# mborhi/CoMA-UNet

Hardware: AMD Instinct MI355X
Metric: volumes/sec (train fwd+bwd) at 128^3 bf16 (higher is better)
Workload: dtype bf16; 1 GPU; CoMA-UNet train step (fwd + RoiMSE/RnC loss + bwd + all-reduce + AdamW), 128^3 volumes, batch 2/GPU, 6-dim covariates (BASELINE configs[3]); global_batch=2, parallelism=dp1, launch=hipGraph replay of the whole step

## Files before the change

coma_unet_amd/csrc/conv_mfma.hip:

```cpp
#include "conv_mfma.h"
#include <type_traits>

template <typename T> struct elem;
template <> struct elem<bf16_t> { static constexpr int EPB = 8; };
template <> struct elem<float> { static constexpr int EPB = 4; };

__device__ __forceinline__ f32x16_t mma_piece(const uint4& a, const uint4& b, f32x16_t acc, bf16_t) {
  return __builtin_amdgcn_mfma_f32_32x32x16_bf16(*reinterpret_cast<const bf16x8_t*>(&a), *reinterpret_cast<const bf16x8_t*>(&b), acc, 0, 0, 0);
}
__device__ __forceinline__ f32x16_t mma_piece(const uint4& a, const uint4& b, f32x16_t acc, float) {
  acc = __builtin_amdgcn_mfma_f32_32x32x2f32(__uint_as_float(a.x), __uint_as_float(b.x), acc, 0, 0, 0);
  acc = __builtin_amdgcn_mfma_f32_32x32x2f32(__uint_as_float(a.y), __uint_as_float(b.y), acc, 0, 0, 0);
  acc = __builtin_amdgcn_mfma_f32_32x32x2f32(__uint_as_float(a.z), __uint_as_float(b.z), acc, 0, 0, 0);
  acc = __builtin_amdgcn_mfma_f32_32x32x2f32(__uint_as_float(a.w), __uint_as_float(b.w), acc, 0, 0, 0);
  return acc;
}

struct GatherP {
  const void* x; int ldx; long sbx; int Di, Hi, Wi, C;
  void* y; int ldy; long sby; int Do, Ho, Wo, N;
  const void* w; long wsb;
  const float* bias; int bsb;
  int k, stride, flip;
  int Mz, My, Mx;
  int ksplit;
  float* part; long part_sb;
  int accum;
  double2* stats; int stats_inst;
};

__device__ __forceinline__ int swz(int row, int chunk) { return (row << 2) | (chunk ^ ((row >> 2) & 3)); }

template <int BN, int MODE, typename T = bf16_t>
__global__ __launch_bounds__(256, 2) void conv_mfma_gather_k(GatherP p) {
  constexpr int EPB = elem<T>::EPB, CKL = 4 * EPB, LCK = EPB == 8 ? 5 : 4;
  constexpr int BM = (BN == 128) ? 128 : 256;
  constexpr int WAVES_N = (BN == 128) ? 2 : 1;
  constexpr int NT = BN / 32 / WAVES_N;
  constexpr int MT = 2;
  constexpr int A_PIECES = BM * 4 / 256;
  constexpr int B_PIECES = (BN * 4 + 255) / 256;
  extern __shared__ __attribute__((aligned(16))) char smem[];
  uint4* ldsA = reinterpret_cast<uint4*>(smem);
  uint4* ldsB = ldsA + 2 * BM * 4;
  int* rowoff = reinterpret_cast<int*>(ldsB + 2 * BN * 4);

  const int tid = threadIdx.x, lane = tid & 63, wid = tid >> 6;
  const int wm = wid / WAVES_N, wn = wid % WAVES_N;
  const int b = blockIdx.z;
  int nblk, cls = 0, ysl = blockIdx.y, ksi = 0;
  if (p.ksplit > 1) { ksi = ysl % p.ksplit; ysl /= p.ksplit; }
  if (MODE == 1) { cls = ysl & 7; nblk = ysl >> 3; } else { nblk = ysl; }
  const int n0 = nblk * BN;
  const int pz = (cls >> 2) & 1, py = (cls >> 1) & 1, px = cls & 1;
  const long Mtot = (long)p.Mz * p.My * p.Mx;
  const long m0 = (long)blockIdx.x * BM;
  const T* xb = static_cast<const T*>(p.x) + (long)b * p.sbx;
  const T* wb = static_cast<const T*>(p.w) + (long)b * p.wsb;
  const int pad = (p.k - 1) >> 1;

  const int chunk = tid & 3;
  int rz[A_PIECES], ry[A_PIECES], rx[A_PIECES];
#pragma unroll
  for (int i = 0; i < A_PIECES; ++i) {
    const int row = (tid >> 2) + 64 * i;
    const long m = m0 + row;
    if (m < Mtot) {
      const int mx = (int)(m % p.Mx), my = (int)((m / p.Mx) % p.My), mz = (int)(m / ((long)p.Mx * p.My));
      if (MODE == 0) { rz[i] = mz * p.stride - pad; ry[i] = my * p.stride - pad; rx[i] = mx * p.stride - pad; }
      else { rz[i] = mz; ry[i] = my; rx[i] = mx; }
      if (chunk == 0) {
        int off;
        if (MODE == 0) off = (int)(m * p.ldy);
        else {
          const int oz = 2 * mz + pz, oy = 2 * my + py, ox = 2 * mx + px;
          off = (oz < p.Do && oy < p.Ho && ox < p.Wo) ? (((oz * p.Ho + oy) * p.Wo + ox) * p.ldy) : -1;
        }
        rowoff[row] = off;
      }
    } else {
      rz[i] = ry[i] = rx[i] = -(1 << 20);
      if (chunk == 0) rowoff[row] = -1;
    }
  }

  const int cchunks = p.C >> LCK;
  int ntaps;
  if (MODE == 0) ntaps = p.k * p.k * p.k; else ntaps = (1 + pz) * (1 + py) * (1 + px);
  const int nsteps_all = ntaps * cchunks;
  const int s_begin = p.ksplit > 1 ? (int)((long)nsteps_all * ksi / p.ksplit) : 0;
  const int s_end = p.ksplit > 1 ? (int)((long)nsteps_all * (ksi + 1) / p.ksplit) : nsteps_all;
  const int nsteps = s_end - s_begin;
  if (nsteps <= 0) return;

  uint4 ra[A_PIECES], rb[B_PIECES];
  const int l_nx = MODE == 0 ? p.k : 1 + px, l_ny = MODE == 0 ? p.k : 1 + py;
  int l_t = s_begin / cchunks, l_cc = s_begin % cchunks;
  int l_jx = l_t % l_nx, l_jy = (l_t / l_nx) % l_ny, l_jz = l_t / (l_nx * l_ny);
  auto load_step = [&](int) {
    const int t = l_t, cc = l_cc;
    int dz, dy, dx, wtap;
    if (MODE == 0) {
      dz = l_jz; dy = l_jy; dx = l_jx;
      wtap = p.flip ? (ntaps - 1 - t) : t;
    } else {
      const int jx = l_jx, jy = l_jy, jz = l_jz;
      const int tx = px ? (jx ? 2 : 0) : 1, ty = py ? (jy ? 2 : 0) : 1, tz = pz ? (jz ? 2 : 0) : 1;
      dx = px ? (jx ? 0 : 1) : 0; dy = py ? (jy ? 0 : 1) : 0; dz = pz ? (jz ? 0 : 1) : 0;
      wtap = (tz * 3 + ty) * 3 + tx;
    }
    const int c0 = cc * CKL + chunk * EPB;
#pragma unroll
    for (int i = 0; i < A_PIECES; ++i) {
      const int iz = rz[i] + dz, iy = ry[i] + dy, ix = rx[i] + dx;
      const bool ok = (unsigned)iz < (unsigned)p.Di && (unsigned)iy < (unsigned)p.Hi && (unsigned)ix < (unsigned)p.Wi;
      ra[i] = make_uint4(0, 0, 0, 0);
      if (ok) ra[i] = *reinterpret_cast<const uint4*>(xb + (long)((iz * p.Hi + iy) * p.Wi + ix) * p.ldx + c0);
    }
#pragma unroll
    for (int i = 0; i < B_PIECES; ++i) {
      const int piece = tid + 256 * i;
      const int n = piece >> 2;
      rb[i] = make_uint4(0, 0, 0, 0);
      if (n < BN) rb[i] = *reinterpret_cast<const uint4*>(wb + ((long)wtap * p.N + n0 + n) * p.C + c0);
    }
    if (++l_cc == cchunks) {
      l_cc = 0; ++l_t;
      if (++l_jx == l_nx) { l_jx = 0; if (++l_jy == l_ny) { l_jy = 0; ++l_jz; } }
    }
  };
  auto store_step = [&](int buf) {
#pragma unroll
    for (int i = 0; i < A_PIECES; ++i) ldsA[buf * BM * 4 + swz((tid >> 2) + 64 * i, chunk)] = ra[i];
#pragma unroll
    for (int i = 0; i < B_PIECES; ++i) {
      const int piece = tid + 256 * i;
      const int n = piece >> 2;
      if (n < BN) ldsB[buf * BN * 4 + swz(n, chunk)] = rb[i];
    }
  };

  f32x16_t acc[MT][NT];
#pragma unroll
  for (int i = 0; i < MT; ++i)
#pragma unroll
    for (int j = 0; j < NT; ++j)
#pragma unroll
      for (int e = 0; e < 16; ++e) acc[i][j][e] = 0.f;

  load_step(0);
  store_step(0);
  __syncthreads();
  const int fr = lane & 31, fh = lane >> 5;
  int cur = 0;
  for (int step = 0; step < nsteps; ++step) {
    if (step + 1 < nsteps) load_step(step + 1);
    const uint4* A = ldsA + cur * BM * 4;
    const uint4* B = ldsB + cur * BN * 4;
#pragma unroll
    for (int ks = 0; ks < 2; ++ks) {
      uint4 af[MT], bfr[NT];
#pragma unroll
      for (int i = 0; i < MT; ++i) af[i] = A[swz(wm * 64 + i * 32 + fr, ks * 2 + fh)];
#pragma unroll
      for (int j = 0; j < NT; ++j) bfr[j] = B[swz(wn * (NT * 32) + j * 32 + fr, ks * 2 + fh)];
#pragma unroll
      for (int i = 0; i < MT; ++i)
#pragma unroll
        for (int j = 0; j < NT; ++j) acc[i][j] = mma_piece(af[i], bfr[j], acc[i][j], T());
    }
    if (step + 1 < nsteps) store_step(cur ^ 1);
    __syncthreads();
    cur ^= 1;
  }

  T* yb = static_cast<T*>(p.y) + (long)b * p.sby;
  const bool do_stats = p.stats != nullptr;
  float st_s[NT], st_q[NT];
#pragma unroll
  for (int j = 0; j < NT; ++j) {
    const int n = n0 + wn * (NT * 32) + j * 32 + fr;
    const float bv = p.bias ? p.bias[b * p.bsb + n] : 0.f;
    st_s[j] = 0.f; st_q[j] = 0.f;
#pragma unroll
    for (int i = 0; i < MT; ++i) {
#pragma unroll
      for (int e = 0; e < 16; ++e) {
        const int row = wm * 64 + i * 32 + (e & 3) + 8 * (e >> 2) + 4 * fh;
        const int off = rowoff[row];
        if (off >= 0) {
          if (p.ksplit > 1) atomicAdd(p.part + (long)b * p.part_sb + (long)(off / p.ldy) * p.N + n, acc[i][j][e]);
          else {
            const T o = static_cast<T>(acc[i][j][e] + bv + (p.accum ? static_cast<float>(yb[off + n]) : 0.f));
            yb[off + n] = o;
            if (do_stats) { const float r = static_cast<float>(o); st_s[j] += r; st_q[j] = fmaf(r, r, st_q[j]); }
          }
        }
      }
    }
  }
  if (do_stats) {
    __syncthreads();
    float* red = reinterpret_cast<float*>(smem);
#pragma unroll
    for (int j = 0; j < NT; ++j) {
      float a = st_s[j], c = st_q[j];
      a += __shfl_xor(a, 32, 64); c += __shfl_xor(c, 32, 64);
      if (fh == 0) { red[((wid * NT + j) * 32 + fr) * 2] = a; red[((wid * NT + j) * 32 + fr) * 2 + 1] = c; }
    }
    __syncthreads();
    for (int t = tid; t < BN; t += 256) {
      const int twn = t / (NT * 32), tj = (t / 32) % NT, tfr = t & 31;
      double a = 0.0, c = 0.0;
      for (int w = 0; w < 4 / WAVES_N; ++w) {
        const int wv_ = w * WAVES_N + twn;
        a += (double)red[((wv_ * NT + tj) * 32 + tfr) * 2]; c += (double)red[((wv_ * NT + tj) * 32 + tfr) * 2 + 1];
      }
      stat_add(p.stats, p.stats_inst ? p.stats_inst : 1, p.N, p.stats_inst ? b : 0, n0 + t, a, c);
    }
  }
}

template <typename T>
__global__ __launch_bounds__(256) void gather_finalize_k(const float* __restrict__ part, long part_sb, T* __restrict__ y, int ldy,
                                                         long sby, int N, long V, const float* __restrict__ bias, int bsb, int accum) {
  const int b = blockIdx.y;
  const long total = V * N;
  for (long e = (long)blockIdx.x * 256 + threadIdx.x; e < total; e += (long)gridDim.x * 256) {
    const long v = e / N; const int n = (int)(e - v * N);
    T* dst = y + (long)b * sby + v * ldy + n;
    *dst = static_cast<T>(part[(long)b * part_sb + e] + (bias ? bias[b * bsb + n] : 0.f) + (accum ? static_cast<float>(*dst) : 0.f));
  }
}

struct HaloP {
  const void* x; int ldx; long sbx; int D, H, W, C;
  void* y; int ldy; long sby; int N;
  const void* w; long wsb;
  const float* bias; int bsb;
  int flip, vecx, vecw;
  int ntx, nty, ntz;
};

template <int CPR> __device__ __forceinline__ int hswz(int row, int chunk) {
  if (CPR == 4) return (row << 2) | (chunk ^ ((row >> 2) & 3));
  return (row << 1) | (chunk ^ ((row >> 3) & 1));
}

template <int CK, int LX, int VEC, typename T = bf16_t>
__global__ __launch_bounds__(256, 2) void conv_mfma_halo_k(HaloP p) {
  constexpr int EPB = elem<T>::EPB;
  static_assert(EPB == 8 || VEC == 1, "fp32 staging is vector-only");
  constexpr int TX = 1 << LX, RY = 32 / TX;
  constexpr int TY = 4 * RY, TZ = 2;
  constexpr int HX = TX + 2, HY = TY + 2, HZ = TZ + 2, HV = HX * HY * HZ;
  constexpr int CPR = CK / EPB;
  constexpr int KS = CPR / 2;
  extern __shared__ __attribute__((aligned(16))) char smem[];
  uint4* Hl = reinterpret_cast<uint4*>(smem);
  uint4* Wl = Hl + HV * CPR;
  const int tid = threadIdx.x, lane = tid & 63, wid = tid >> 6;
  const int b = blockIdx.z, n0 = blockIdx.y * 32;
  int tix, tiy, tiz;
  if (!tile_coords(xcd_remap(blockIdx.x, gridDim.x), p.ntx, p.nty, p.ntz, tix, tiy, tiz)) return;
  const int x0 = tix * TX, y0 = tiy * TY, z0 = tiz * TZ;
  const T* xb = static_cast<const T*>(p.x) + (long)b * p.sbx;
  const T* wb = static_cast<const T*>(p.w) + (long)b * p.wsb;
  const int fr = lane & 31, fh = lane >> 5;

  f32x16_t acc[2];
#pragma unroll
  for (int i = 0; i < 2; ++i)
#pragma unroll
    for (int e = 0; e < 16; ++e) acc[i][e] = 0.f;
// ... 1888 lines not shown
  TconvP q;
  q.x = x->data; q.ldx = (int)x->ld; q.sbx = x->sb; q.D = x->D; q.H = x->H; q.W = x->W; q.C = x->C;
  q.y = y->data; q.ldy = (int)y->ld; q.sby = y->sb; q.Do = y->D; q.Ho = y->H; q.Wo = y->W; q.N = y->C;
  q.w = wk; q.wsb = d->per_sample_w ? 27L * y->C * x->C : 0;
  q.bias = bias; q.bsb = d->per_sample_w ? y->C : 0;
  q.xbytes = (unsigned)((unsigned long long)t_vox(x) * x->ld * sizeof(T));
  q.wbytes = (unsigned)(27ull * y->C * x->C * sizeof(T));
  q.accum = accum;
  const int nblk_n = y->C / 32;
  const TileRun r = tile_run(q.D, q.H, q.W, 32, 4, 2, 512, nblk_n * x->B);
  q.ntx = r.ntx; q.nty = r.nty; q.ntz = r.ntz; q.ids_total = r.ids_total; q.ids_per_block = r.ids_per_block;
  q.stats = nullptr; q.stats_inst = stats_inst;
  static const bool fuse_stats = getenv("COMA_TCONV_NO_STATS") == nullptr;
  if (stats && !accum && fuse_stats) { q.stats = stats; *stats_chunks = 1; }
  const size_t lds = (size_t)(33 * 5 * 3 + 14 * 32) * 80;
  coma_set_kernel_tag("conv_mfma_tconv_k<%s, %d>", sizeof(T) == 2 ? "__bf16" : "float", q.stats ? 1 : 0);
  const dim3 grid((unsigned)r.gx, (unsigned)nblk_n, (unsigned)x->B);
  if (q.stats) { set_max_lds<conv_mfma_tconv_k<T, true>>(); hipLaunchKernelGGL((conv_mfma_tconv_k<T, true>), grid, dim3(256), lds, s, q); }
  else { set_max_lds<conv_mfma_tconv_k<T, false>>(); hipLaunchKernelGGL((conv_mfma_tconv_k<T, false>), grid, dim3(256), lds, s, q); }
  COMA_LAUNCH_CHECK();
  return 0;
}

bool conv_mfma_supported(const coma_conv_desc* d, const coma_tensor* x, const coma_tensor* y) {
  if (x->dtype != COMA_BF16 || y->dtype != COMA_BF16) return false;
  if ((long)t_vox(x) * x->ld >= (1L << 31) || (long)t_vox(y) * y->ld >= (1L << 31)) return false;
  if (halo_ok(d, x, y)) return true;
  if (pw_ok(d, x, y)) return true;
  if (x->C % 32 || y->C % 32) return false;
  if (x->ld % 8 || y->ld % 8 || x->sb % 8 || y->sb % 8) return false;
  if (x->data && !aligned16(x->data)) return false;
  if ((long)t_vox(x) * x->ld >= (1L << 31) || (long)t_vox(y) * y->ld >= (1L << 31)) return false;
  if (d->form == 1 && d->stride == 2 && d->ksize != 3) return false;
  return true;
}

static bool f32_halo_ok(const coma_conv_desc* d, const coma_tensor* x, const coma_tensor* y) {
  if (x->W < 16 && x->C % 32 == 0 && y->C % 32 == 0) return false;
  return d->ksize == 3 && d->stride == 1 && x->W >= 8 && (long)x->H * x->W >= 32 && x->C % 16 == 0 && y->C >= 16 &&
         x->ld % 4 == 0 && x->sb % 4 == 0 && (!x->data || aligned16(x->data)) && (unsigned long long)t_vox(x) * x->ld * 4 < 0x7fff0000ull;
}
bool conv_f32mfma_supported(const coma_conv_desc* d, const coma_tensor* x, const coma_tensor* y) {
  if (x->dtype != COMA_F32 || y->dtype != COMA_F32) return false;
  if ((long)t_vox(x) * x->ld >= (1L << 31) || (long)t_vox(y) * y->ld >= (1L << 31)) return false;
  if (thin16f_ok(d, x, y)) return true;
  if (f32_halo_ok(d, x, y)) return true;
  if (x->C % 16 || y->C % 32) return false;
  if (x->ld % 4 || y->ld % 4 || x->sb % 4 || y->sb % 4) return false;
  if (x->data && !aligned16(x->data)) return false;
  if (d->form == 1 && d->stride == 2 && d->ksize != 3) return false;
  return true;
}

static int gather_ksplit(long blocks, int nsteps, bool f32) {
  if (f32) {
    if (blocks >= 192 || nsteps < 8) return 1;
    long ks = 256 / blocks;
    if (ks > 8) ks = 8;
    if (ks > nsteps / 4) ks = nsteps / 4;
    return ks < 2 ? 1 : (int)ks;
  }
  if (blocks >= 384 || nsteps < 16) return 1;
  long ks = 512 / blocks;
  if (ks > 8) ks = 8;
  if (ks > nsteps / 4) ks = nsteps / 4;
  return ks < 2 ? 1 : (int)ks;
}

struct GatherGrid { long gx, gy; int ksplit; };
static GatherGrid gather_grid(int BN, int mode, long Mtot, int N, int B, int taps, int C, bool f32) {
  const int BM = BN == 128 ? 128 : 256, LCK = f32 ? 4 : 5;
  GatherGrid g;
  g.gx = (Mtot + BM - 1) / BM; g.gy = (long)(N / BN) * (mode == 1 ? 8 : 1);
  g.ksplit = gather_ksplit(g.gx * g.gy * B, (mode == 1 ? 1 : taps) * (C >> LCK), f32);
  return g;
}

template <int BN, typename T>
static int launch_gather(const GatherP& p0, int mode, int B, hipStream_t s, void* ws, size_t ws_bytes, int ws_zeroed,
                         double2* stats, int stats_inst, int* stats_chunks) {
  GatherP p = p0;
  constexpr int BM = (BN == 128) ? 128 : 256;
  constexpr int LCK = elem<T>::EPB == 8 ? 5 : 4;
  const size_t lds = (size_t)2 * (BM + BN) * 64 + BM * 4;
  const GatherGrid g = gather_grid(BN, mode, (long)p.Mz * p.My * p.Mx, p.N, B, p.k * p.k * p.k, p.C, LCK == 4);
  const unsigned gx = (unsigned)g.gx, gy = (unsigned)g.gy;
  const long Vout = (long)p.Do * p.Ho * p.Wo;
  p.ksplit = g.ksplit;
  p.part = nullptr; p.part_sb = 0;
  if (p.ksplit > 1 && ws && ws_bytes >= sizeof(float) * (size_t)B * Vout * p.N) {
    p.part = (float*)ws; p.part_sb = Vout * p.N;
    if (!ws_zeroed && hipMemsetAsync(ws, 0, sizeof(float) * (size_t)B * Vout * p.N, s) != hipSuccess) { coma_set_error("conv split-K memset failed"); return 2; }
  } else p.ksplit = 1;
  p.stats = nullptr; p.stats_inst = stats_inst;
  if (stats && p.ksplit == 1 && !p.accum) { p.stats = stats; *stats_chunks = 1; }
  dim3 grid(gx, gy * p.ksplit, (unsigned)B);
  coma_set_kernel_tag("conv_mfma_gather_k<%d, %d, %s>", BN, mode, LCK == 4 ? "float" : "__bf16");
  if (mode == 0) hipLaunchKernelGGL((conv_mfma_gather_k<BN, 0, T>), grid, dim3(256), lds, s, p);
  else hipLaunchKernelGGL((conv_mfma_gather_k<BN, 1, T>), grid, dim3(256), lds, s, p);
  COMA_LAUNCH_CHECK();
  if (p.ksplit > 1) {
    long nb = (Vout * p.N + 255) / 256;
    if (nb > 1024) nb = 1024;
    hipLaunchKernelGGL(gather_finalize_k<T>, dim3((unsigned)nb, (unsigned)B), dim3(256), 0, s, (const float*)p.part, p.part_sb, (T*)p.y, p.ldy,
                       p.sby, p.N, Vout, p.bias, p.bsb, p.accum);
    COMA_LAUNCH_CHECK();
  }
  return 0;
}

template <int CK, int LX, int VEC, typename T>
static int launch_halo(const HaloP& p0, int B, hipStream_t s) {
  HaloP p = p0;
  constexpr int TX = 1 << LX, RY = 32 / TX, TY = 4 * RY, TZ = 2;
  constexpr int HV = (TX + 2) * (TY + 2) * (TZ + 2);
  p.ntx = (p.W + TX - 1) / TX; p.nty = (p.H + TY - 1) / TY; p.ntz = (p.D + TZ - 1) / TZ;
  const size_t lds = (size_t)(HV + 9 * 32) * CK * sizeof(T);
  set_max_lds<conv_mfma_halo_k<CK, LX, VEC, T>, 96>();
  dim3 grid((unsigned)(p.ntx * p.nty * ((p.ntz + 7) / 8) * 8), (unsigned)((p.N + 31) / 32), (unsigned)B);
  coma_set_kernel_tag("conv_mfma_halo_k<%d, %d, %d, %s>", CK, LX, VEC, sizeof(T) == 4 ? "float" : "__bf16");
  hipLaunchKernelGGL((conv_mfma_halo_k<CK, LX, VEC, T>), grid, dim3(256), lds, s, p);
  COMA_LAUNCH_CHECK();
  return 0;
}

static int duo_mode() {
  static const int mode = getenv("COMA_NO_DUO") != nullptr ? 0 : getenv("COMA_DUO_C32_ONLY") != nullptr ? 1 : 2;
  return mode;
}
static size_t duo_frag_bytes(const coma_conv_desc* d, const coma_tensor* x, const coma_tensor* y) {
  if (duo_mode() < 2 || x->dtype != COMA_BF16 || d->ksize != 3 || d->stride != 1 || x->W < 16) return 0;
  if (x->C < 64 || x->C % 16 || y->C % 32) return 0;
  return (size_t)(d->per_sample_w ? x->B : 1) * 27 * y->C * x->C * 2;
}

static bool duo_wide_ok(const coma_conv_desc* d, const coma_tensor* x, const coma_tensor* y) {
  if (duo_frag_bytes(d, x, y) == 0 || x->C <= 32 || x->C % 32) return false;
  const bool vecx = x->ld % 8 == 0 && x->sb % 8 == 0 && aligned16(x->data);
  const bool st16 = y->ld % 8 == 0 && y->sb % 8 == 0 && aligned16(y->data);
  return vecx && st16 && (unsigned long long)t_vox(x) * x->ld * sizeof(bf16_t) < 0x7fff0000ull &&
         x->D <= 510 && x->H <= 510 && x->W <= 510;
}

template <typename T>
static int conv_mfma_halo(const coma_conv_desc* d, const coma_tensor* x, const void* wk, const float* bias,
                          const coma_tensor* y, hipStream_t s, double2* stats = nullptr, int stats_inst = 0,
                          int* stats_chunks = nullptr, void* ws = nullptr, size_t ws_bytes = 0, bool wk_frag = false) {
  constexpr int EPB = elem<T>::EPB;
  constexpr bool F32 = EPB == 4;
  HaloP p;
  p.x = x->data; p.ldx = (int)x->ld; p.sbx = x->sb; p.D = x->D; p.H = x->H; p.W = x->W; p.C = x->C;
  p.y = y->data; p.ldy = (int)y->ld; p.sby = y->sb; p.N = y->C;
  p.w = wk; p.wsb = d->per_sample_w ? 27L * y->C * x->C : 0;
  p.bias = bias; p.bsb = d->per_sample_w ? y->C : 0;
  p.flip = d->form == 1;
  p.vecx = x->ld % EPB == 0 && x->sb % EPB == 0 && aligned16(x->data);
  p.vecw = x->C % EPB == 0 && aligned16(wk);
  const bool thin = !F32 && x->C <= 16;
  const int lx = x->W >= 32 ? 5 : (x->W >= 16 ? 4 : 3);
  const bool vec = p.vecx && p.vecw && x->C % (4 * EPB) == 0 && (unsigned long long)t_vox(x) * x->ld * sizeof(T) < 0x7fff0000ull;
  if (F32) COMA_CHECK(vec, "conv_mfma(fp32): operands must allow 16-byte channel pieces (C %% 16 == 0, aligned)");
  if constexpr (!F32) {
    static const bool thin16_on = []{ const char* e = getenv("COMA_THIN16"); return !(e && e[0] == '0'); }();
    const unsigned long long xb_ = (unsigned long long)t_vox(x) * x->ld * sizeof(T);
    if (thin16_on && thin && lx == 5 && y->C <= (x->C > 8 ? 16 : 32) && p.vecx && xb_ < 0x7fff0000ull) {
      Thin16P q;
      q.x = (const bf16_t*)p.x; q.ldx = p.ldx; q.sbx = p.sbx; q.D = p.D; q.H = p.H; q.W = p.W; q.C = p.C;
      q.y = (bf16_t*)p.y; q.ldy = p.ldy; q.sby = p.sby; q.N = p.N; q.w = (const bf16_t*)p.w; q.wsb = p.wsb; q.bias = p.bias; q.bsb = p.bsb;
      q.flip = p.flip; q.xbytes = (unsigned)xb_;
      q.st8 = y->ld % 4 == 0 && y->sb % 4 == 0 && (((uintptr_t)y->data) & 7) == 0;
      const TileRun r = tile_run(q.D, q.H, q.W, 32, 4, 2, 1024, x->B);
      q.ntx = r.ntx; q.nty = r.nty; q.ntz = r.ntz; q.ids_total = r.ids_total; q.ids_per_block = r.ids_per_block;
      q.stats = nullptr; q.stats_inst = stats_inst;
      if (stats) { q.stats = stats; *stats_chunks = 1; }
      dim3 grid((unsigned)r.gx, 1, (unsigned)x->B);
      const bool c16 = q.C > 8, n32 = q.N > 16;
      size_t lds = (size_t)34 * 6 * 4 * (c16 ? 32 : 16);
      if (lds < (size_t)27 * q.N * q.C * 2) lds = (size_t)27 * q.N * q.C * 2;
      coma_set_kernel_tag("conv_thin16_k<%d, %d>", c16 ? 16 : 8, n32 ? 2 : 1);
      if (c16) hipLaunchKernelGGL((conv_thin16_k<16, 1>), grid, dim3(256), lds, s, q);
      else     { if (n32) hipLaunchKernelGGL((conv_thin16_k<8, 2>), grid, dim3(256), lds, s, q);  else hipLaunchKernelGGL((conv_thin16_k<8, 1>), grid, dim3(256), lds, s, q); }
      COMA_LAUNCH_CHECK();
// ... 87 lines not shown
    }
    if (vec) {
      if (lx == 5) return launch_halo<32, 5, 1, bf16_t>(p, x->B, s);
      if (lx == 4) return launch_halo<32, 4, 1, bf16_t>(p, x->B, s);
      return launch_halo<32, 3, 1, bf16_t>(p, x->B, s);
    }
    if (lx == 5) return launch_halo<32, 5, 0, bf16_t>(p, x->B, s);
    if (lx == 4) return launch_halo<32, 4, 0, bf16_t>(p, x->B, s);
    return launch_halo<32, 3, 0, bf16_t>(p, x->B, s);
  }
}

bool conv_mfma_accumulate_ok(const coma_conv_desc* d, const coma_tensor* x, const coma_tensor* y) {
  if (x->dtype == COMA_F32) return conv_f32mfma_supported(d, x, y) && !thin16f_ok(d, x, y) && !f32_halo_ok(d, x, y);
  return conv_mfma_supported(d, x, y) && !halo_ok(d, x, y);
}

size_t conv_mfma_wk_frag_bytes(const coma_conv_desc* d, const coma_tensor* x, const coma_tensor* y) {
  if (x->dtype != COMA_BF16 || y->dtype != COMA_BF16 || !conv_mfma_supported(d, x, y) || !halo_ok(d, x, y) || !duo_wide_ok(d, x, y)) return 0;
  return duo_frag_bytes(d, x, y);
}

size_t conv_mfma_fwd_ws_bytes(const coma_conv_desc* d, const coma_tensor* x, const coma_tensor* y) {
  if (x->dtype == COMA_F32) { if (thin16f_ok(d, x, y) || f32_halo_ok(d, x, y)) return 0; }
  else if (halo_ok(d, x, y)) return duo_frag_bytes(d, x, y);
  else if (pw_ok(d, x, y)) return 0;
  if (tconv_ok(d, x, y)) return 0;
  const size_t bytes = sizeof(float) * (size_t)y->B * t_vox(y) * y->C;
  if (bytes > ((size_t)64 << 20)) return 0;
  const int BN = y->C % 128 == 0 ? 128 : y->C % 64 == 0 ? 64 : 32;
  const int mode = d->form == 1 && d->stride == 2;
  const long Mtot = mode ? (long)((y->D + 1) / 2) * ((y->H + 1) / 2) * ((y->W + 1) / 2) : (long)t_vox(y);
  return gather_grid(BN, mode, Mtot, y->C, y->B, d->ksize * d->ksize * d->ksize, x->C, x->dtype == COMA_F32).ksplit > 1 ? bytes : 0;
}

int conv_mfma_fwd(const coma_conv_desc* d, const coma_tensor* x, const void* wk, const float* bias,
                  const coma_tensor* y, hipStream_t s, double2* stats, int stats_inst, int* stats_chunks, void* ws,
                  size_t ws_bytes, int ws_zeroed, int accum, int wk_frag) {
  const bool f32 = x->dtype == COMA_F32;
  if (wk_frag) {
    COMA_CHECK(!accum && aligned16(wk) && conv_mfma_wk_frag_bytes(d, x, y) > 0,
               "conv_mfma: COMA_WK_FRAG on a problem the wide two-group kernel does not take (ask coma_conv_wk_frag_bytes)");
    return conv_mfma_halo<bf16_t>(d, x, wk, bias, y, s, stats, stats_inst, stats_chunks, nullptr, 0, true);
  }
  COMA_CHECK(!accum || conv_mfma_accumulate_ok(d, x, y), "conv_mfma: this problem's kernel family cannot accumulate into y");
  if (f32 && thin16f_ok(d, x, y)) return conv_thin16f(d, x, wk, bias, y, s, stats, stats_inst, stats_chunks);
  if (f32) { if (f32_halo_ok(d, x, y)) return conv_mfma_halo<float>(d, x, wk, bias, y, s, stats, stats_inst, stats_chunks); }
  else if (halo_ok(d, x, y)) return conv_mfma_halo<bf16_t>(d, x, wk, bias, y, s, stats, stats_inst, stats_chunks, ws, ws_bytes);
  if (tconv_ok(d, x, y)) {
    if (f32) return conv_mfma_tconv<float>(d, x, wk, bias, y, s, stats, stats_inst, stats_chunks, accum);
    return conv_mfma_tconv<bf16_t>(d, x, wk, bias, y, s, stats, stats_inst, stats_chunks, accum);
  }
  if (!f32 && pw_ok(d, x, y) && !(x->C % 32 == 0 && y->C % 32 == 0 && x->C * y->C > 64 * 32)) {
    COMA_CHECK(aligned16(wk), "conv_mfma: weights must be 16-byte aligned");
    PwP q;
    q.x = (const bf16_t*)x->data; q.ldx = (int)x->ld; q.sbx = x->sb; q.V = t_vox(x); q.C = x->C;
    q.y = (bf16_t*)y->data; q.ldy = (int)y->ld; q.sby = y->sb; q.N = y->C;
    q.w = (const bf16_t*)wk; q.wsb = d->per_sample_w ? (long)y->C * x->C : 0;
    q.bias = bias; q.bsb = d->per_sample_w ? y->C : 0;
    q.st8 = y->ld % 4 == 0 && y->sb % 4 == 0 && (((uintptr_t)y->data) & 7) == 0;
    q.st16 = y->ld % 8 == 0 && y->sb % 8 == 0 && (((uintptr_t)y->data) & 15) == 0;
    const int ks = (x->C + 15) / 16, nt = (y->C + 31) / 32;
    long nb = ((q.V + 31) / 32 + 3) / 4;
    if (nb > 2048) nb = 2048;
    q.stats = nullptr; q.stats_inst = stats_inst; q.accum = accum;
    if (stats) { q.stats = stats; *stats_chunks = 1; }
    dim3 grid((unsigned)nb, (unsigned)x->B);
    coma_set_kernel_tag("conv_mfma_pw_k<%d, %d>", ks > 4 ? 4 : ks, nt);
#define PWL(K_, N_) hipLaunchKernelGGL((conv_mfma_pw_k<K_, N_>), grid, dim3(256), 0, s, q)
    if (nt == 1) { if (ks == 1) PWL(1, 1); else if (ks == 2) PWL(2, 1); else if (ks == 3) PWL(3, 1); else PWL(4, 1); }
    else { if (ks == 1) PWL(1, 2); else if (ks == 2) PWL(2, 2); else if (ks == 3) PWL(3, 2); else PWL(4, 2); }
#undef PWL
    COMA_LAUNCH_CHECK();
    return 0;
  }
  COMA_CHECK(aligned16(wk) && aligned16(x->data), "conv_mfma: operands must be 16-byte aligned");
  GatherP p;
  p.x = x->data; p.ldx = (int)x->ld; p.sbx = x->sb; p.Di = x->D; p.Hi = x->H; p.Wi = x->W; p.C = x->C;
  p.y = y->data; p.ldy = (int)y->ld; p.sby = y->sb; p.Do = y->D; p.Ho = y->H; p.Wo = y->W; p.N = y->C;
  const int taps = d->ksize * d->ksize * d->ksize;
  p.w = wk; p.wsb = d->per_sample_w ? (long)taps * y->C * x->C : 0;
  p.bias = bias; p.bsb = d->per_sample_w ? y->C : 0;
  p.k = d->ksize; p.stride = d->stride; p.flip = 0; p.accum = accum;
  int mode = 0;
  if (d->form == 1 && d->stride == 1) { p.flip = 1; }
  if (d->form == 1 && d->stride == 2) {
    mode = 1;
    p.Mz = (y->D + 1) / 2; p.My = (y->H + 1) / 2; p.Mx = (y->W + 1) / 2;
  } else {
    p.Mz = y->D; p.My = y->H; p.Mx = y->W;
  }
  if (f32) {
    if (y->C % 128 == 0) return launch_gather<128, float>(p, mode, x->B, s, ws, ws_bytes, ws_zeroed, stats, stats_inst, stats_chunks);
    if (y->C % 64 == 0) return launch_gather<64, float>(p, mode, x->B, s, ws, ws_bytes, ws_zeroed, stats, stats_inst, stats_chunks);
    return launch_gather<32, float>(p, mode, x->B, s, ws, ws_bytes, ws_zeroed, stats, stats_inst, stats_chunks);
  }
  if (y->C % 128 == 0) return launch_gather<128, bf16_t>(p, mode, x->B, s, ws, ws_bytes, ws_zeroed, stats, stats_inst, stats_chunks);
  if (y->C % 64 == 0) return launch_gather<64, bf16_t>(p, mode, x->B, s, ws, ws_bytes, ws_zeroed, stats, stats_inst, stats_chunks);
  return launch_gather<32, bf16_t>(p, mode, x->B, s, ws, ws_bytes, ws_zeroed, stats, stats_inst, stats_chunks);
}

struct Wgrad2P {
  const bf16_t* dyp; int ldn; long sbn;
  const bf16_t* xp; int ldc; long sbc;
  int N, C, D, H, W;
  int ntx, nty, ntz, tiles_total, tiles_per_block, cblocks;
  int vec_n, vec_c;
  int lgd, lgg;
  float* dwk; long wsb;
  int nrep; long rep_stride;
};

template <int HX, int HY, int NT>
__device__ __forceinline__ void wgrad2_tile(const char* Dt, const char* Gt, int lane_d, int lane_g, const int (&toff)[NT],
                                            int ntap, f32x16_t (&acc)[NT], int ks0, int ksd) {
  constexpr int PD = 64, PG = 64;
  auto rd_d = [&](int ks) -> bf16x8_t {
    const int z = ks >> 3, y = (ks >> 1) & 3, xh = ks & 1;
    const char* dp = Dt + lane_d + ((z * 4 + y) * 32 + xh * 16) * PD;
    const s4_t dlo = __builtin_amdgcn_ds_read_tr16_b64_v4i16((lds_s4_t*)(dp));
    const s4_t dhi = __builtin_amdgcn_ds_read_tr16_b64_v4i16((lds_s4_t*)(dp + 4 * PD));
    return (bf16x8_t){dlo[0], dlo[1], dlo[2], dlo[3], dhi[0], dhi[1], dhi[2], dhi[3]};
  };
  auto rd_g = [&](int ks, int t) -> bf16x8_t {
    const int z = ks >> 3, y = (ks >> 1) & 3, xh = ks & 1;
    const char* gp = Gt + lane_g + ((z * HY + y) * HX + xh * 16) * PG;
    const s4_t glo = __builtin_amdgcn_ds_read_tr16_b64_v4i16((lds_s4_t*)(gp + toff[t]));
    const s4_t ghi = __builtin_amdgcn_ds_read_tr16_b64_v4i16((lds_s4_t*)(gp + toff[t] + 4 * PG));
    return (bf16x8_t){glo[0], glo[1], glo[2], glo[3], ghi[0], ghi[1], ghi[2], ghi[3]};
  };
  (void)ntap;
  bf16x8_t df = rd_d(ks0), gf = rd_g(ks0, 0);
#pragma unroll 2
  for (int ks = ks0; ks < 16; ks += ksd) {
    const int kn = ks + ksd < 16 ? ks + ksd : ks;
    bf16x8_t dn = df;
#pragma unroll
    for (int t = 0; t < NT; ++t) {
      bf16x8_t gn;
      if (t + 1 < NT) gn = rd_g(ks, t + 1);
      else { dn = rd_d(kn); gn = rd_g(kn, 0); }
      __builtin_amdgcn_sched_barrier(0);
      acc[t] = __builtin_amdgcn_mfma_f32_32x32x16_bf16(df, gf, acc[t], 0, 0, 0);
      __builtin_amdgcn_sched_barrier(0);
      gf = gn;
    }
    df = dn;
  }
}

template <int VEC, int OCC, int K, int PK>
__global__ __launch_bounds__(256, OCC) void conv_mfma_wgrad2_k(Wgrad2P p) {
  constexpr int PADK = (K - 1) / 2;
  constexpr int NTILE = K == 1 ? 1 : (PK == 1 ? 27 : PK == 2 ? 18 : 9), NT = (NTILE + 3) / 4;
  constexpr int TX = 32, TY = 4, TZ = 2, TM = TX * TY * TZ, HX = TX + K - 1, HY = TY + K - 1, HZ = TZ + K - 1, HV = HX * HY * HZ;
  constexpr int NDP = TM * 4, NGP = HV * 4;
  constexpr int DIT = NDP / 256, GIT = (NGP + 255) / 256;
  extern __shared__ __attribute__((aligned(16))) char smem[];
  char* Dt = smem;
  char* Gt = smem + TM * 64;
  const int tid = threadIdx.x, lane = tid & 63;
  const int wid = __builtin_amdgcn_readfirstlane(tid >> 6);
  const int b = blockIdx.z;
  const int nb = blockIdx.y / p.cblocks, cb = blockIdx.y % p.cblocks;
  const int n0 = nb * 32, c0 = cb * 32;
  const bf16_t* dyb = p.dyp + (long)b * p.sbn + n0;
// ... 954 lines not shown
```

Measured before the change: 120.4 volumes/s.

## Use buffer loads with precomputed tap masks and two-step LDS pipelining in gather conv

Moves the gather implicit-GEMM conv kernel's global loads to raw buffer loads. Out-of-range taps are handled by sending the offset past the buffer range, using per-row bitmasks computed once, so the per-step bounds arithmetic goes away. The main loop now stages two K-steps per LDS buffer and doubles LDS to four images, halving the barrier count and deepening prefetch. The cost is more registers (two register sets of loads) and more LDS, which may lower occupancy. Offsets are limited to 32 bits and kernel size to at most 9.

```diff
diff --git a/coma_unet_amd/csrc/conv_mfma.hip b/coma_unet_amd/csrc/conv_mfma.hip
--- a/coma_unet_amd/csrc/conv_mfma.hip
+++ b/coma_unet_amd/csrc/conv_mfma.hip
@@ -20,6 +20,7 @@
   const void* x; int ldx; long sbx; int Di, Hi, Wi, C;
   void* y; int ldy; long sby; int Do, Ho, Wo, N;
   const void* w; long wsb;
+  unsigned xbytes, wbytes;
   const float* bias; int bsb;
   int k, stride, flip;
   int Mz, My, Mx;
@@ -40,10 +41,12 @@
   constexpr int MT = 2;
   constexpr int A_PIECES = BM * 4 / 256;
   constexpr int B_PIECES = (BN * 4 + 255) / 256;
+  constexpr int SA = BM * 4, SB = BN * 4;
+  typedef unsigned g_u32x4_t __attribute__((ext_vector_type(4)));
   extern __shared__ __attribute__((aligned(16))) char smem[];
-  uint4* ldsA = reinterpret_cast<uint4*>(smem);
-  uint4* ldsB = ldsA + 2 * BM * 4;
-  int* rowoff = reinterpret_cast<int*>(ldsB + 2 * BN * 4);
+  g_u32x4_t* ldsA = reinterpret_cast<g_u32x4_t*>(smem);
+  g_u32x4_t* ldsB = ldsA + 4 * SA;
+  int* rowoff = reinterpret_cast<int*>(smem);
 
   const int tid = threadIdx.x, lane = tid & 63, wid = tid >> 6;
   const int wm = wid / WAVES_N, wn = wid % WAVES_N;
@@ -60,27 +63,35 @@
   const int pad = (p.k - 1) >> 1;
 
   const int chunk = tid & 3;
-  int rz[A_PIECES], ry[A_PIECES], rx[A_PIECES];
+  unsigned a_boff[A_PIECES], a_in[A_PIECES];
+  int roff[A_PIECES];
+  const int out_ld = p.ksplit > 1 ? p.N : p.ldy;
+  auto in_mask = [&](int r, int par, int D) -> unsigned {
+    if (MODE == 0) {
+      const int lo = r < 0 ? -r : 0, hi = D - 1 - r < p.k - 1 ? D - 1 - r : p.k - 1;
+      return hi >= lo ? (2u << hi) - (1u << lo) : 0u;
+    }
+    const unsigned here = (unsigned)r < (unsigned)D, next = (unsigned)(r + 1) < (unsigned)D;
+    return par ? (next | here << 1) : here;
+  };
 #pragma unroll
   for (int i = 0; i < A_PIECES; ++i) {
     const int row = (tid >> 2) + 64 * i;
     const long m = m0 + row;
+    a_boff[i] = 0; a_in[i] = 0; roff[i] = -1;
     if (m < Mtot) {
-      const int mx = (int)(m % p.Mx), my = (int)((m / p.Mx) % p.My), mz = (int)(m / ((long)p.Mx * p.My));
-      if (MODE == 0) { rz[i] = mz * p.stride - pad; ry[i] = my * p.stride - pad; rx[i] = mx * p.stride - pad; }
-      else { rz[i] = mz; ry[i] = my; rx[i] = mx; }
-      if (chunk == 0) {
-        int off;
-        if (MODE == 0) off = (int)(m * p.ldy);
-        else {
-          const int oz = 2 * mz + pz, oy = 2 * my + py, ox = 2 * mx + px;
-          off = (oz < p.Do && oy < p.Ho && ox < p.Wo) ? (((oz * p.Ho + oy) * p.Wo + ox) * p.ldy) : -1;
-        }
-        rowoff[row] = off;
-      }
-    } else {
-      rz[i] = ry[i] = rx[i] = -(1 << 20);
-      if (chunk == 0) rowoff[row] = -1;
+      const unsigned mq = (unsigned)m / (unsigned)p.Mx;
+      const int mx = (int)((unsigned)m - mq * (unsigned)p.Mx), mz = (int)(mq / (unsigned)p.My), my = (int)(mq - (unsigned)mz * (unsigned)p.My);
+      int rz, ry, rx;
+      if (MODE == 0) { rz = mz * p.stride - pad; ry = my * p.stride - pad; rx = mx * p.stride - pad; }
+      else { rz = mz; ry = my; rx = mx; }
+      a_boff[i] = (unsigned)((rz * p.Hi + ry) * p.Wi + rx) * (unsigned)(p.ldx * (int)sizeof(T)) + (unsigned)(chunk * 16);
+      a_in[i] = in_mask(rz, pz, p.Di) | in_mask(ry, py, p.Hi) << 10 | in_mask(rx, px, p.Wi) << 20;
+      if (MODE == 0) roff[i] = (int)m * out_ld;
+      else {
+        const int oz = 2 * mz + pz, oy = 2 * my + py, ox = 2 * mx + px;
+        roff[i] = (oz < p.Do && oy < p.Ho && ox < p.Wo) ? (((oz * p.Ho + oy) * p.Wo + ox) * out_ld) : -1;
+      }
     }
   }
 
@@ -93,11 +104,25 @@
   const int nsteps = s_end - s_begin;
   if (nsteps <= 0) return;
 
-  uint4 ra[A_PIECES], rb[B_PIECES];
+  const __amdgpu_buffer_rsrc_t rs_x = __builtin_amdgcn_make_buffer_rsrc(const_cast<T*>(xb), 0, p.xbytes, 0x00020000);
+  const __amdgpu_buffer_rsrc_t rs_w = __builtin_amdgcn_make_buffer_rsrc(const_cast<T*>(wb), 0, p.wbytes, 0x00020000);
+  constexpr unsigned OOB = 0x7fff0000u;
+  unsigned w_boff[B_PIECES];
+#pragma unroll
+  for (int i = 0; i < B_PIECES; ++i) {
+    const int n = (tid + 256 * i) >> 2;
+    w_boff[i] = n < BN ? (unsigned)(((n0 + n) * p.C + chunk * EPB) * (int)sizeof(T)) : OOB;
+  }
+  const unsigned w_tap = (unsigned)(p.N * p.C * (int)sizeof(T));
+
+  g_u32x4_t ra[2][A_PIECES], rb[2][B_PIECES];
   const int l_nx = MODE == 0 ? p.k : 1 + px, l_ny = MODE == 0 ? p.k : 1 + py;
   int l_t = s_begin / cchunks, l_cc = s_begin % cchunks;
   int l_jx = l_t % l_nx, l_jy = (l_t / l_nx) % l_ny, l_jz = l_t / (l_nx * l_ny);
-  auto load_step = [&](int) {
+  typedef std::integral_constant<int, 0> first_t;
+  typedef std::integral_constant<int, 1> second_t;
+  auto load_step = [&](auto half_c) {
+    constexpr int half = decltype(half_c)::value;
     const int t = l_t, cc = l_cc;
     int dz, dy, dx, wtap;
     if (MODE == 0) {
@@ -109,34 +134,33 @@
       dx = px ? (jx ? 0 : 1) : 0; dy = py ? (jy ? 0 : 1) : 0; dz = pz ? (jz ? 0 : 1) : 0;
       wtap = (tz * 3 + ty) * 3 + tx;
     }
-    const int c0 = cc * CKL + chunk * EPB;
-#pragma unroll
-    for (int i = 0; i < A_PIECES; ++i) {
-      const int iz = rz[i] + dz, iy = ry[i] + dy, ix = rx[i] + dx;
-      const bool ok = (unsigned)iz < (unsigned)p.Di && (unsigned)iy < (unsigned)p.Hi && (unsigned)ix < (unsigned)p.Wi;
-      ra[i] = make_uint4(0, 0, 0, 0);
-      if (ok) ra[i] = *reinterpret_cast<const uint4*>(xb + (long)((iz * p.Hi + iy) * p.Wi + ix) * p.ldx + c0);
-    }
-#pragma unroll
-    for (int i = 0; i < B_PIECES; ++i) {
-      const int piece = tid + 256 * i;
-      const int n = piece >> 2;
-      rb[i] = make_uint4(0, 0, 0, 0);
-      if (n < BN) rb[i] = *reinterpret_cast<const uint4*>(wb + ((long)wtap * p.N + n0 + n) * p.C + c0);
-    }
+    const unsigned step_b = (unsigned)((dz * p.Hi + dy) * p.Wi + dx) * (unsigned)(p.ldx * (int)sizeof(T)) + (unsigned)(cc * 64);
+    const unsigned need = 1u << l_jz | 1u << (10 + l_jy) | 1u << (20 + l_jx);
+#pragma unroll
+    for (int i = 0; i < A_PIECES; ++i)
+      ra[half][i] = __builtin_amdgcn_raw_buffer_load_b128(rs_x, (a_in[i] & need) == need ? a_boff[i] + step_b : OOB, 0, 0);
+    const int w_b = (int)((unsigned)wtap * w_tap + (unsigned)(cc * CKL * (int)sizeof(T)));
+#pragma unroll
+    for (int i = 0; i < B_PIECES; ++i) rb[half][i] = __builtin_amdgcn_raw_buffer_load_b128(rs_w, w_boff[i], w_b, 0);
     if (++l_cc == cchunks) {
       l_cc = 0; ++l_t;
       if (++l_jx == l_nx) { l_jx = 0; if (++l_jy == l_ny) { l_jy = 0; ++l_jz; } }
     }
   };
-  auto store_step = [&](int buf) {
-#pragma unroll
-    for (int i = 0; i < A_PIECES; ++i) ldsA[buf * BM * 4 + swz((tid >> 2) + 64 * i, chunk)] = ra[i];
-#pragma unroll
-    for (int i = 0; i < B_PIECES; ++i) {
-      const int piece = tid + 256 * i;
-      const int n = piece >> 2;
-      if (n < BN) ldsB[buf * BN * 4 + swz(n, chunk)] = rb[i];
+  auto load_pair = [&](int pair) {
+    load_step(first_t());
+    if (2 * pair + 1 < nsteps) load_step(second_t());
+  };
+  auto store_pair = [&](int buf) {
+#pragma unroll
+    for (int h = 0; h < 2; ++h) {
+#pragma unroll
+      for (int i = 0; i < A_PIECES; ++i) ldsA[(buf * 2 + h) * SA + swz((tid >> 2) + 64 * i, chunk)] = ra[h][i];
+#pragma unroll
+      for (int i = 0; i < B_PIECES; ++i) {
+        const int n = (tid + 256 * i) >> 2;
+        if (n < BN) ldsB[(buf * 2 + h) * SB + swz(n, chunk)] = rb[h][i];
+      }
     }
   };
 
@@ -148,31 +172,48 @@
 #pragma unroll
       for (int e = 0; e < 16; ++e) acc[i][j][e] = 0.f;
 
-  load_step(0);
-  store_step(0);
+  const int fr = lane & 31, fh = lane >> 5;
+  auto mma_step = [&](int img) {
+    const g_u32x4_t* A = ldsA + img * SA;
+    const g_u32x4_t* B = ldsB + img * SB;
+#pragma unroll
+    for (int ks = 0; ks < 2; ++ks) {
+      g_u32x4_t af[MT], bfr[NT];
+#pragma unroll
+      for (int i = 0; i < MT; ++i) af[i] = A[swz(wm * 64 + i * 32 + fr, ks * 2 + fh)];
+#pragma unroll
+      for (int j = 0; j < NT; ++j) bfr[j] = B[swz(wn * (NT * 32) + j * 32 + fr, ks * 2 + fh)];
+#pragma unroll
+      for (int i = 0; i < MT; ++i)
+#pragma unroll
+        for (int j = 0; j < NT; ++j)
+          acc[i][j] = mma_piece(reinterpret_cast<const uint4&>(af[i]), reinterpret_cast<const uint4&>(bfr[j]), acc[i][j], T());
+    }
+  };
+
+#pragma unroll
+  for (int i = 0; i < A_PIECES; ++i) ra[1][i] = g_u32x4_t{0u, 0u, 0u, 0u};
+#pragma unroll
+  for (int i = 0; i < B_PIECES; ++i) rb[1][i] = g_u32x4_t{0u, 0u, 0u, 0u};
+  const int npairs = (nsteps + 1) >> 1;
+  load_pair(0);
+  store_pair(0);
+  if (npairs > 1) load_pair(1);
   __syncthreads();
-  const int fr = lane & 31, fh = lane >> 5;
-  int cur = 0;
-  for (int step = 0; step < nsteps; ++step) {
-    if (step + 1 < nsteps) load_step(step + 1);
-    const uint4* A = ldsA + cur * BM * 4;
-    const uint4* B = ldsB + cur * BN * 4;
-#pragma unroll
-    for (int ks = 0; ks < 2; ++ks) {
-      uint4 af[MT], bfr[NT];
-#pragma unroll
-      for (int i = 0; i < MT; ++i) af[i] = A[swz(wm * 64 + i * 32 + fr, ks * 2 + fh)];
-#pragma unroll
-      for (int j = 0; j < NT; ++j) bfr[j] = B[swz(wn * (NT * 32) + j * 32 + fr, ks * 2 + fh)];
-#pragma unroll
-      for (int i = 0; i < MT; ++i)
-#pragma unroll
-        for (int j = 0; j < NT; ++j) acc[i][j] = mma_piece(af[i], bfr[j], acc[i][j], T());
-    }
-    if (step + 1 < nsteps) store_step(cur ^ 1);
+  for (int pair = 0; pair < npairs; ++pair) {
+    const int cur = pair & 1;
+    if (pair + 1 < npairs) {
+      store_pair(cur ^ 1);
+      if (pair + 2 < npairs) load_pair(pair + 2);
+    }
+    mma_step(2 * cur);
+    if (2 * pair + 1 < nsteps) mma_step(2 * cur + 1);
     __syncthreads();
-    cur ^= 1;
-  }
+  }
+#pragma unroll
+  for (int i = 0; i < A_PIECES; ++i)
+    if (chunk == 0) rowoff[(tid >> 2) + 64 * i] = roff[i];
+  __syncthreads();
 
   T* yb = static_cast<T*>(p.y) + (long)b * p.sby;
   const bool do_stats = p.stats != nullptr;
@@ -189,7 +230,7 @@
         const int row = wm * 64 + i * 32 + (e & 3) + 8 * (e >> 2) + 4 * fh;
         const int off = rowoff[row];
         if (off >= 0) {
-          if (p.ksplit > 1) atomicAdd(p.part + (long)b * p.part_sb + (long)(off / p.ldy) * p.N + n, acc[i][j][e]);
+          if (p.ksplit > 1) atomicAdd(p.part + (long)b * p.part_sb + off + n, acc[i][j][e]);
           else {
             const T o = static_cast<T>(acc[i][j][e] + bv + (p.accum ? static_cast<float>(yb[off + n]) : 0.f));
             yb[off + n] = o;
@@ -2244,7 +2285,7 @@
   GatherP p = p0;
   constexpr int BM = (BN == 128) ? 128 : 256;
   constexpr int LCK = elem<T>::EPB == 8 ? 5 : 4;
-  const size_t lds = (size_t)2 * (BM + BN) * 64 + BM * 4;
+  const size_t lds = (size_t)4 * (BM + BN) * 64;
   const GatherGrid g = gather_grid(BN, mode, (long)p.Mz * p.My * p.Mx, p.N, B, p.k * p.k * p.k, p.C, LCK == 4);
   const unsigned gx = (unsigned)g.gx, gy = (unsigned)g.gy;
   const long Vout = (long)p.Do * p.Ho * p.Wo;
@@ -2258,8 +2299,8 @@
   if (stats && p.ksplit == 1 && !p.accum) { p.stats = stats; *stats_chunks = 1; }
   dim3 grid(gx, gy * p.ksplit, (unsigned)B);
   coma_set_kernel_tag("conv_mfma_gather_k<%d, %d, %s>", BN, mode, LCK == 4 ? "float" : "__bf16");
-  if (mode == 0) hipLaunchKernelGGL((conv_mfma_gather_k<BN, 0, T>), grid, dim3(256), lds, s, p);
-  else hipLaunchKernelGGL((conv_mfma_gather_k<BN, 1, T>), grid, dim3(256), lds, s, p);
+  if (mode == 0) { set_max_lds<conv_mfma_gather_k<BN, 0, T>, 80>(); hipLaunchKernelGGL((conv_mfma_gather_k<BN, 0, T>), grid, dim3(256), lds, s, p); }
+  else { set_max_lds<conv_mfma_gather_k<BN, 1, T>, 80>(); hipLaunchKernelGGL((conv_mfma_gather_k<BN, 1, T>), grid, dim3(256), lds, s, p); }
   COMA_LAUNCH_CHECK();
   if (p.ksplit > 1) {
     long nb = (Vout * p.N + 255) / 256;
@@ -2513,6 +2554,13 @@
   p.w = wk; p.wsb = d->per_sample_w ? (long)taps * y->C * x->C : 0;
   p.bias = bias; p.bsb = d->per_sample_w ? y->C : 0;
   p.k = d->ksize; p.stride = d->stride; p.flip = 0; p.accum = accum;
+  {
+    const unsigned long long esz = f32 ? 4 : 2;
+    const unsigned long long xb_ = ((unsigned long long)(t_vox(x) - 1) * x->ld + x->C) * esz, wb_ = (unsigned long long)taps * y->C * x->C * esz;
+    COMA_CHECK(d->ksize <= 9 && xb_ <= 0x7fff0000ull && wb_ <= 0x7fff0000ull,
+               "conv_mfma: gather kernel takes kernel sizes up to 9 and up to 0x7fff0000 bytes per sample of x and per weight set");
+    p.xbytes = (unsigned)xb_; p.wbytes = (unsigned)wb_;
+  }
   int mode = 0;
   if (d->form == 1 && d->stride == 1) { p.flip = 1; }
   if (d->form == 1 && d->stride == 2) {
```

Result: no change. 121.2 volumes/s, median of 6 (+0.7%).
